# hugocornellier/face_detection_tflite

Measured on NVIDIA B200. Metric: images/sec BlazeFace detect (pre+infer+NMS), higher is better.
Workload: dtype f32

## Files before the change

face_detection_tflite_b200/csrc/engine.cu:

```cuda
#include "engine.h"

#include <algorithm>
#include <cstdio>
#include <cstdlib>

namespace fdt {

Engine::~Engine() {
  if (d_blob_) cudaFree(d_blob_);
  for (TailLayerD* p : d_tail_) if (p) cudaFree(p);
  for (TailBlk* p : d_blks_) if (p) cudaFree(p);
}

bool Engine::init(const uint8_t* tflite, size_t len, int fuse_level, std::string* err, bool use_tc) {
  if (!model_.parse(tflite, len, err)) return false;
  if (!plan_.build(model_, fuse_level, err, use_tc)) return false;
  size_t bytes = plan_.blob.size() * sizeof(float) + 64;
  if (cudaMalloc(&d_blob_, bytes) != cudaSuccess) { *err = "cudaMalloc(weights) failed"; return false; }
  cudaMemset(d_blob_, 0, bytes);
  if (cudaMemcpy(d_blob_, plan_.blob.data(), plan_.blob.size() * sizeof(float), cudaMemcpyHostToDevice) != cudaSuccess) {
    *err = "weight upload failed";
    return false;
  }
  d_tail_.assign(plan_.steps.size(), nullptr);
// ... 193 lines not shown
        p.no = st.no; p.KSo = st.KSo; p.out_stage_floats = st.out_stage_floats;
        p.out2 = nullptr; p.out2_istride = 0; p.Cs2 = 0; p.c1 = 0; p.c2 = 0;
        if (st.out2 >= 0) {
          TV o2 = view(ctx, st.out2);
          p.out2 = o2.p; p.out2_istride = o2.istride; p.Cs2 = o2.Cs; p.c1 = st.c1; p.c2 = st.c2;
          p.Cout = st.c1;
        }
        p.in_floats = st.in_stage_floats;
        if (!launch_block_ws(p, B, ctx.cap, s)) { failed_ = true; fprintf(stderr, "fdt: k_block_ws could not be launched for step '%s'\n", st.name.c_str()); }
        break;
      }
      case kStepTailWs: {
        TailP p;
        TV iv = view(ctx, st.in);
        p.in = iv.p; p.in_istride = iv.istride; p.H = iv.H; p.W = iv.W; p.CinS = iv.Cs;
        p.blob = blob; p.layers = d_tail_[&st - plan_.steps.data()]; p.nlayers = (int)st.tail.size();
        p.nbuf = st.tail_nbuf;
        for (int k = 0; k < kTailMaxBufs; ++k) { p.buf_off[k] = st.tail_buf_off[k]; p.buf_ks[k] = st.tail_buf_ks[k]; }
        p.act_floats = st.tail_act_floats; p.in_bytes = st.tail_in_bytes;
        p.generic = 0;
        for (const TailLayerD& L : st.tail)
          if (L.kind >= 2 || L.act == 2 || L.w_parts != 1 || L.wscale != 1.f || L.rbuf != L.src || (L.kind != 1 && L.o1 >= 0)) p.generic = 1;
        p.blks = nullptr; p.nblks = 0; p.bias_floats = 0; p.in_px = iv.H * iv.W;
        for (int k = 0; k < 2; ++k) { p.rsrc[k] = nullptr; p.rs_istride[k] = 0; p.rs_cs[k] = p.rs_w[k] = p.rs_c[k] = 0; }
        if (st.tail_wide) {
          p.generic = 2;
          p.blks = d_blks_[&st - plan_.steps.data()]; p.nblks = (int)st.tail_blks.size(); p.bias_floats = st.tail_bias_floats;
          for (size_t k = 0; k < st.tail_rsrc.size() && k < 2; ++k) {
            TV rv = view(ctx, st.tail_rsrc[k]);
            p.rsrc[k] = rv.p; p.rs_istride[k] = rv.istride; p.rs_cs[k] = rv.Cs; p.rs_w[k] = rv.W; p.rs_c[k] = rv.C;
          }
        }
        p.last_a_layer = st.tail_last_a; p.wbuf_bytes = st.tail_wbuf; p.wdepth = st.tail_wdepth; p.tbuf_bytes = st.tail_tbuf; p.smem_bytes = st.smem;
        for (int k = 0; k < 4; ++k) { p.outs[k] = nullptr; p.out_istride[k] = 0; p.out_pix[k] = 0; }
        for (size_t k = 0; k < st.tail_outs.size(); ++k) {
          TV ov = view(ctx, st.tail_outs[k]);
          p.outs[k] = ov.p; p.out_istride[k] = ov.istride; p.out_pix[k] = ov.Cs;
        }
        if (!launch_tail_ws(p, B, ctx.cap, s)) { failed_ = true; fprintf(stderr, "fdt: k_tail_ws could not be launched for step '%s'\n", st.name.c_str()); }
        break;
      }
      case kStepFcTc: {
        FcP p;
        TV iv = view(ctx, st.in);
        p.in = iv.p; p.in_istride = iv.istride;
        p.out = out.p; p.out_istride = out.istride;
        p.w = blob + st.w; p.bias = blob + st.bias;
        p.K = st.K; p.K16 = st.K8; p.N = st.Cout; p.w_parts = st.w_parts; p.tile_bytes = st.ts_rec_bytes; p.wscale = (float)st.out_scale;
        if (!launch_fc_tc(p, B, s)) { failed_ = true; fprintf(stderr, "fdt: k_fc_tc could not be launched for step '%s'\n", st.name.c_str()); }
        break;
      }
      case kStepBlockTs: {
        BlockTsP p;
        TV iv = view(ctx, st.in);
        p.in = iv.p; p.in_istride = iv.istride; p.H = iv.H; p.W = iv.W; p.CinS = iv.Cs;
        p.out = out.p; p.out_istride = out.istride; p.OH = out.H; p.OW = out.W; p.CoutS = out.Cs;
        p.rec = blob + st.ts_rec; p.bias = blob + st.ts_bias; p.rec_bytes = st.ts_rec_bytes;
        p.Cin = iv.C; p.K16 = st.ts_k16; p.Npad = st.ts_npad; p.KS = st.ts_ks;
        p.stride = st.dws; p.res = st.ts_res; p.relu = st.ts_relu;
        p.wide = (out.Cs % 8 == 0 && out.istride % 8 == 0 && ((size_t)out.p % 32 == 0)) ? 1 : 0;
        p.ns = st.ts_ns; p.stage_bytes = st.ts_stage_bytes; p.smem_bytes = st.smem;
        {
          const float* hdw = plan_.blob.data() + st.ts_rec + (size_t)st.ts_npad * st.ts_k16 / 2;
          for (int q = 0; q < 16; ++q)
            for (int k = 0; k < 10; ++k)
              for (int c = 0; c < 4; ++c) p.dw[(q * 10 + k) * 4 + c] = 4 * q + c < st.ts_k16 ? hdw[k * st.ts_k16 + 4 * q + c] : 0.f;
// ... 40 lines not shown
```

face_detection_tflite_b200/csrc/kernels.h:

```cpp
#pragma once
#include <cuda_runtime.h>
#include <algorithm>
#include <cstdint>

#include "../../include/fdt_api.h"
#include "tail_layer.h"

namespace fdt {

enum { kActNone = 0, kActRelu = 1, kActPrelu = 2 };

struct FastDiv {
  unsigned mul = 0, shr = 0, d = 1;
  FastDiv() {}
  explicit FastDiv(int div) {
    d = div < 1 ? 1u : (unsigned)div;
    unsigned l = 0;
    while ((1ull << l) < d) ++l;
    shr = l;
    mul = (unsigned)(((1ull << 32) * ((1ull << l) - d)) / d + 1);
  }
#ifdef __CUDACC__
  __device__ __forceinline__ int div(int n) const { return (int)((__umulhi(mul, (unsigned)n) + (unsigned)n) >> shr); }
  __device__ __forceinline__ void divmod(int n, int& q, int& r) const { q = div(n); r = n - q * (int)d; }
// ... 148 lines not shown
  float* out; long long out_istride; int OH, OW, CoutS;
  const float* rec;
  const float* bias;
  int rec_bytes;
  int Cin, K16, Npad, KS;
  int stride;
  int res;
  int relu, wide;
  int ns, stage_bytes;
  size_t smem_bytes;
  alignas(16) float dw[10 * 64];
};
size_t ts_smem_bytes(int rec_bytes, int Npad, int ns, int stage_bytes);
bool launch_block_ts(const BlockTsP& p, int B, int cap, cudaStream_t s);

struct TailP {
  const float* in; long long in_istride; int H, W, CinS;
  const float* blob;
  const TailLayerD* layers;
  int nlayers;
  int nbuf;
  int buf_off[kTailMaxBufs];
  int buf_ks[kTailMaxBufs];
  int act_floats;
  int in_bytes;
  int last_a_layer;
  int wbuf_bytes, wdepth;
  int tbuf_bytes;
  int generic;
  const TailBlk* blks; int nblks; int bias_floats; int in_px;
  const float* rsrc[2]; long long rs_istride[2]; int rs_cs[2], rs_w[2], rs_c[2];
  float* outs[4]; long long out_istride[4]; int out_pix[4];
  size_t smem_bytes;
};
size_t tail_smem_bytes(int act_floats, int wbuf_bytes, int wdepth, int tbuf_bytes);
size_t wide_smem_bytes(int act_floats, int wbuf_bytes, int wdepth, int tbuf_bytes, int bias_floats);
bool launch_tail_ws(const TailP& p, int B, int cap, cudaStream_t s);

struct FcP {
  const float* in; long long in_istride;
  float* out; long long out_istride;
  const float* w;
  const float* bias;
  int K, K16, N, w_parts, tile_bytes;
  float wscale;
};
bool launch_fc_tc(const FcP& p, int B, cudaStream_t s);

struct JpegIdctP {
  const int16_t* coef;
  const uint16_t* q;
  int bw, bh;
  uint8_t* plane; int pitch;
};
struct JpegColorP {
  const uint8_t* py; const uint8_t* pcb; const uint8_t* pcr;
  int pitch_y, pitch_c;
  int W, H, ncomp;
  int cdw, cdh, hs, vs;
  int orientation;
  uint8_t* out; int out_w;
};
void launch_jpeg_idct(const JpegIdctP& p, cudaStream_t s);
void launch_jpeg_color(const JpegColorP& p, cudaStream_t s);

struct DecodeP {
// ... 55 lines not shown
```

face_detection_tflite_b200/csrc/kernels_tail.cu:

```cuda
#include <cuda.h>
#include <cuda_fp16.h>

#include <algorithm>
#include <cstdio>
#include <map>
#include <mutex>
#include <tuple>

#include "kernels.h"

namespace fdt {
namespace {

#ifndef FDT_TAIL_WARPS
#define FDT_TAIL_WARPS 12
#endif
constexpr int kTC = FDT_TAIL_WARPS;
constexpr int kTG = kTC / 4;
constexpr int kTComputeThreads = kTC * 32;
constexpr int kTThreads = (kTC + 1) * 32;
__device__ __forceinline__ uint32_t col_d(int t) { return t ? 128u : 0u; }
__device__ __forceinline__ uint32_t col_a(int t) { return t ? 384u : 256u; }
constexpr uint32_t kLBO = 128;

// ... 25 lines not shown
}
__device__ __forceinline__ void fma4(float4& a, const float4& v, const float4& w) {
  asm("{\n\t.reg .b64 ra, rv, rw;\n\t"
      "mov.b64 ra, {%0, %1};\n\tmov.b64 rv, {%4, %5};\n\tmov.b64 rw, {%8, %9};\n\t"
      "fma.rn.f32x2 ra, rv, rw, ra;\n\tmov.b64 {%0, %1}, ra;\n\t"
      "mov.b64 ra, {%2, %3};\n\tmov.b64 rv, {%6, %7};\n\tmov.b64 rw, {%10, %11};\n\t"
      "fma.rn.f32x2 ra, rv, rw, ra;\n\tmov.b64 {%2, %3}, ra;\n\t}"
      : "+f"(a.x), "+f"(a.y), "+f"(a.z), "+f"(a.w)
      : "f"(v.x), "f"(v.y), "f"(v.z), "f"(v.w), "f"(w.x), "f"(w.y), "f"(w.z), "f"(w.w));
}
__device__ __forceinline__ float4 max4(const float4& a, const float4& b) {
  return make_float4(fmaxf(a.x, b.x), fmaxf(a.y, b.y), fmaxf(a.z, b.z), fmaxf(a.w, b.w));
}
__device__ __forceinline__ uint32_t pack_h2(float e0, float e1) {
  uint32_t d;
  asm("cvt.rn.satfinite.f16x2.f32 %0, %1, %2;" : "=r"(d) : "f"(e1), "f"(e0));
  return d;
}
__device__ __forceinline__ void split_store_tmem(uint32_t taddr_hi, const float4& a) {
  const uint32_t h0 = pack_h2(a.x, a.y), h1 = pack_h2(a.z, a.w);
  const __half2 hh0 = *reinterpret_cast<const __half2*>(&h0), hh1 = *reinterpret_cast<const __half2*>(&h1);
  const float2 f0 = __half22float2(hh0), f1 = __half22float2(hh1);
  const uint32_t l0 = pack_h2(a.x - f0.x, a.y - f0.y), l1 = pack_h2(a.z - f1.x, a.w - f1.y);
  asm volatile("tcgen05.st.sync.aligned.32x32b.x2.b32 [%0], {%1, %2};" ::"r"(taddr_hi), "r"(h0), "r"(h1) : "memory");
  asm volatile("tcgen05.st.sync.aligned.32x32b.x2.b32 [%0], {%1, %2};" ::"r"(taddr_hi + 64u), "r"(l0), "r"(l1) : "memory");
}
__device__ __forceinline__ void mma_ts_f16(uint32_t tmem_d, uint32_t tmem_a, uint32_t b_lo, uint32_t b_hi, uint32_t idesc, uint32_t acc) {
  asm volatile(
      "{\n\t.reg .pred p;\n\t.reg .b64 db;\n\tmov.b64 db, {%2, %3};\n\tsetp.ne.b32 p, %5, 0;\n\t"
      "tcgen05.mma.cta_group::1.kind::f16 [%0], [%1], db, %4, p;\n\t}\n" ::"r"(tmem_d), "r"(tmem_a), "r"(b_lo), "r"(b_hi), "r"(idesc), "r"(acc));
}

#ifdef FDT_TAIL_TRACE
#define TT(k) do { if (blockIdx.x == 0 && tid == 0 && it == 1) tt[l * 6 + (k)] = clock64(); } while (0)
#else
#define TT(k) do { } while (0)
#endif
template <bool GEN>
__global__ void __launch_bounds__(kTThreads, 1) k_tail_ws(const __grid_constant__ CUtensorMap tmap, const __grid_constant__ TailP p, int B) {
#ifdef FDT_TAIL_TRACE
  __shared__ long long tt[16 * 6];
#endif
  extern __shared__ __align__(128) unsigned char smem_raw[];
  __shared__ uint32_t tmem_base_s;
  const int tid = threadIdx.x, warp = tid >> 5, lane = tid & 31;
  TailLayerD* sL = reinterpret_cast<TailLayerD*>(smem_raw);
  float* sBias = reinterpret_cast<float*>(smem_raw + kTailMaxLayers * sizeof(TailLayerD));
  float* sAlpha = sBias + kTailMaxLayers * 128;
  uint64_t* bars = reinterpret_cast<uint64_t*>(sAlpha + kTailMaxLayers * 128);
  float* scratch = reinterpret_cast<float*>(bars + 16);
  float* act0 = reinterpret_cast<float*>((reinterpret_cast<uintptr_t>(scratch + 16) + 127) & ~(uintptr_t)127);
  float* zslot = act0 + p.act_floats;
  unsigned char* tring = reinterpret_cast<unsigned char*>((reinterpret_cast<uintptr_t>(zslot + 128) + 127) & ~(uintptr_t)127);
  unsigned char* wring = tring + 2 * (size_t)p.tbuf_bytes;
  const uint32_t bar0 = smem_u32(bars);
  const uint32_t in_full = bar0, a_free = bar0 + 8u, w_full = bar0 + 16u, a_full = bar0 + 32u, d_full = bar0 + 48u, t_full = bar0 + 56u;
  const int nl = p.nlayers;
  const int my_images = blockIdx.x < B ? (B - 1 - (int)blockIdx.x) / (int)gridDim.x + 1 : 0;

  for (int i = tid; i < nl * (int)(sizeof(TailLayerD) / 16); i += kTThreads)
    reinterpret_cast<uint4*>(sL)[i] = reinterpret_cast<const uint4*>(p.layers)[i];
  for (int i = (p.in_bytes >> 2) + tid; i < p.act_floats + 128; i += kTThreads) act0[i] = 0.f;
  if (warp == kTC) {
    if (lane == 0) {
      mbar_init(in_full, 1);
      mbar_init(a_free, kTC);
      for (int i = 0; i < 2; ++i) { mbar_init(w_full + 8u * i, 1); mbar_init(a_full + 8u * i, kTC); mbar_init(t_full + 8u * i, 1); }
      mbar_init(d_full, 1);
      asm volatile("fence.mbarrier_init.release.cluster;" ::: "memory");
      asm volatile("prefetch.tensormap [%0];" ::"l"(&tmap) : "memory");
    }
    __syncwarp();
    asm volatile("tcgen05.alloc.cta_group::1.sync.aligned.shared::cta.b32 [%0], %1;" ::"r"(smem_u32(&tmem_base_s)), "r"(512u));
    asm volatile("tcgen05.relinquish_alloc_permit.cta_group::1.sync.aligned;" ::);
  }
  __syncthreads();
  for (int l = 0; l < nl; ++l)
    for (int i = tid; i < sL[l].Npad; i += kTThreads) {
      sBias[l * 128 + i] = p.blob[(size_t)sL[l].bias_off + i];
      if (GEN && sL[l].act == 2) sAlpha[l * 128 + i] = p.blob[(size_t)sL[l].alpha_off + i];
    }
  asm volatile("tcgen05.fence::before_thread_sync;" ::: "memory");
  __syncthreads();
  asm volatile("tcgen05.fence::after_thread_sync;" ::: "memory");
  const uint32_t tmem_base = tmem_base_s;
  const uint32_t act_a = smem_u32(act0), zero_a = smem_u32(zslot), wring_a = smem_u32(wring), tring_a = smem_u32(tring);

  if (warp < kTC) {
    const int lq = warp & 3, g = warp >> 2;
    const int r = lq * 32 + lane;
    const uint32_t tm_lane = tmem_base + ((uint32_t)(lq * 32) << 16);
    uint32_t ph_d = 0u, ph_t0 = 0u, ph_t1 = 0u;
    int gl = 0, it = 0;
    for (int img = blockIdx.x; img < B; img += gridDim.x, ++it) {
      mbar_wait(in_full, (uint32_t)(it & 1));
      for (int l = 0; l < nl; ++l, ++gl) {
        const TailLayerD L = sL[l];
        TT(0);
        const uint32_t src_a = act_a + 4u * (uint32_t)p.buf_off[L.src], kss_b = 4u * (uint32_t)p.buf_ks[L.src];
        const uint32_t dst_a = L.dst >= 0 ? act_a + 4u * (uint32_t)p.buf_off[L.dst] : 0u, ksd_b = L.dst >= 0 ? 4u * (uint32_t)p.buf_ks[L.dst] : 0u;
        const int src_q = (int)(kss_b >> 4), dst_q = (int)(ksd_b >> 4);
        const int npix = L.OH * L.OW;
        const uint32_t tb_a = tring_a + (uint32_t)(gl & 1) * (uint32_t)p.tbuf_bytes;
        if (L.tap_bytes) {
          if (gl & 1) { mbar_wait(t_full + 8u, ph_t1); ph_t1 ^= 1u; } else { mbar_wait(t_full, ph_t0); ph_t0 ^= 1u; }
        }
        TT(1);
        if (GEN && L.kind == 3) {
          const int n = npix * L.Cin;
          float sacc = 0.f;
          for (int i = tid; i < n; i += kTComputeThreads) {
            const int px = i / L.Cin, c = i - px * L.Cin;
            float a, w;
            asm("ld.shared.f32 %0, [%1];" : "=f"(a) : "r"(src_a + (uint32_t)px * kss_b + 4u * (uint32_t)c) : "memory");
            asm("ld.shared.f32 %0, [%1];" : "=f"(w) : "r"(tb_a + 4u * (uint32_t)i) : "memory");
            sacc = fmaf(a, w, sacc);
          }
#pragma unroll
          for (int o = 16; o > 0; o >>= 1) sacc += __shfl_xor_sync(0xffffffffu, sacc, o);
          if (lane == 0) { scratch[warp] = sacc; mbar_arrive(a_full); mbar_arrive(a_full + 8u); }
          asm volatile("bar.sync 1, %0;" ::"n"(kTComputeThreads) : "memory");
          if (tid == 0) {
            float tot = sBias[l * 128];
            for (int w2 = 0; w2 < kTC; ++w2) tot += scratch[w2];
            p.outs[L.o1][(size_t)img * p.out_istride[L.o1]] = tot;
          }
          asm volatile("bar.sync 1, %0;" ::"n"(kTComputeThreads) : "memory");
          if (l == p.last_a_layer && lane == 0) mbar_arrive(a_free);
          continue;
        }
        const bool paired = npix > 128;
        const int ntiles = paired ? 2 : 1;
        const int rows = paired ? (npix >> 1) : npix;
        const int nq = L.K16 >> 2, nq_real = (L.Cin + 3) >> 2, nq_half = (L.K16 >> 5) << 2;
        const uint32_t dww_a = tb_a, dwb_a = dww_a + 9u * (uint32_t)L.K16 * 4u;
        const uint32_t k16_b = (uint32_t)L.K16 * 4u;
        const uint32_t acol0 = tm_lane + col_a(0), acol1 = tm_lane + col_a(1);
        int oy = r / L.OW;
        const int ox = r - oy * L.OW;
        if (paired) oy *= 2;
        const bool act = r < rows;
        const bool warp_on = lq * 32 < rows;
        const int pix0 = oy * L.OW + ox;
        bool half_done = false;
        if (!warp_on) {
        } else if (L.kind == 0) {
          uint32_t off[12];
          const int iy0 = oy * L.stride - L.pad, ix0 = ox * L.stride - L.pad;
#pragma unroll
          for (int k = 0; k < 12; ++k) {
            const int iy = iy0 + k / 3, ix = ix0 + k % 3;
            const bool ok = act && (unsigned)iy < (unsigned)L.IH && (unsigned)ix < (unsigned)L.IW;
            off[k] = ok ? src_a + (uint32_t)(iy * L.IW + ix) * kss_b : zero_a;
          }
          for (int q = g; q < nq; q += kTG) {
            if (!half_done && q >= nq_half) {
              half_done = true;
              asm volatile("tcgen05.wait::st.sync.aligned;" ::: "memory");
              asm volatile("tcgen05.fence::before_thread_sync;" ::: "memory");
              __syncwarp();
              if (lane == 0) mbar_arrive(a_full);
            }
            float4 a0 = make_float4(0.f, 0.f, 0.f, 0.f), a1 = a0;
            if (q < nq_real) {
              const uint32_t qo = 16u * (uint32_t)q;
              float4 w[9];
#pragma unroll
              for (int k = 0; k < 9; ++k) w[k] = lds4(dww_a + (uint32_t)k * k16_b + qo);
              const float4 bias = lds4(dwb_a + qo);
              float4 v[3];
#pragma unroll
              for (int c = 0; c < 3; ++c) v[c] = lds4(off[c] + qo);
              a0 = bias;
#pragma unroll
              for (int c = 0; c < 3; ++c) fma4(a0, v[c], w[c]);
// ... 26 lines not shown
              asm volatile("tcgen05.fence::before_thread_sync;" ::: "memory");
              __syncwarp();
              if (lane == 0) mbar_arrive(a_full);
            }
            const bool in = q < src_q;
            split_store_tmem(acol0 + 2u * (uint32_t)q, in ? lds4(px0 + 16u * (uint32_t)q) : make_float4(0.f, 0.f, 0.f, 0.f));
            if (paired) split_store_tmem(acol1 + 2u * (uint32_t)q, in ? lds4(px1 + 16u * (uint32_t)q) : make_float4(0.f, 0.f, 0.f, 0.f));
          }
        }
        if (warp_on) asm volatile("tcgen05.wait::st.sync.aligned;" ::: "memory");
        TT(2);
        asm volatile("tcgen05.fence::before_thread_sync;" ::: "memory");
        __syncwarp();
        if (lane == 0) { if (!half_done) mbar_arrive(a_full); mbar_arrive(a_full + 8u); }
        if (warp_on) {
          const uint32_t bias_a = smem_u32(sBias + l * 128), alpha_a = smem_u32(sAlpha + l * 128);
          const uint32_t rsrc_a = GEN ? act_a + 4u * (uint32_t)p.buf_off[L.rbuf] : src_a, ksr_b = GEN ? 4u * (uint32_t)p.buf_ks[L.rbuf] : kss_b;
          const int res_q = (int)(ksr_b >> 4);
          mbar_wait(d_full, ph_d);
          TT(3);
          asm volatile("tcgen05.fence::after_thread_sync;" ::: "memory");
          const uint32_t row_b = (uint32_t)L.IW * ksr_b;
#pragma unroll 1
          for (int t = 0; t < ntiles; ++t) {
            const int pix = pix0 + t * L.OW;
            const uint32_t dcol = tm_lane + col_d(t);
            uint32_t res_a = zero_a;
            if (act && L.res == 1) res_a = rsrc_a + (uint32_t)pix * ksr_b;
            if (act && L.res == 2) res_a = rsrc_a + (uint32_t)((2 * oy) * L.IW + 2 * ox) * ksr_b;
            const uint32_t out_a = dst_a + (uint32_t)(act ? pix : 0) * ksd_b;
            float* o1 = nullptr; float* o2 = nullptr;
            int o1_q = 0;
            if (GEN ? L.o1 >= 0 : L.kind == 1) {
              o1 = p.outs[L.o1] + (size_t)img * p.out_istride[L.o1] + (size_t)(act ? pix : 0) * p.out_pix[L.o1];
              o1_q = p.out_pix[L.o1] >> 2;
              if (L.o2 >= 0) o2 = p.outs[L.o2] + (size_t)img * p.out_istride[L.o2] + (size_t)(act ? pix : 0) * p.out_pix[L.o2];
            }
            for (int c16 = g; c16 < (L.Npad >> 4); c16 += kTG) {
              uint32_t u[16];
              asm volatile(
                  "tcgen05.ld.sync.aligned.32x32b.x16.b32 {%0, %1, %2, %3, %4, %5, %6, %7, %8, %9, %10, %11, %12, %13, %14, %15}, [%16];"
                  : "=r"(u[0]), "=r"(u[1]), "=r"(u[2]), "=r"(u[3]), "=r"(u[4]), "=r"(u[5]), "=r"(u[6]), "=r"(u[7]),
                    "=r"(u[8]), "=r"(u[9]), "=r"(u[10]), "=r"(u[11]), "=r"(u[12]), "=r"(u[13]), "=r"(u[14]), "=r"(u[15])
                  : "r"(dcol + 16u * (uint32_t)c16));
              float4 bv[4], rv[4];
#pragma unroll
              for (int j = 0; j < 4; ++j) {
                const int cq = 4 * c16 + j;
                const uint32_t qo = 16u * (uint32_t)cq;
                bv[j] = lds4(bias_a + qo);
                rv[j] = make_float4(0.f, 0.f, 0.f, 0.f);
                if (L.res == 1) {
                  if (cq < res_q) rv[j] = lds4(res_a + qo);
                } else if (L.res == 2) {
                  if (cq < res_q) rv[j] = max4(max4(lds4(res_a + qo), lds4(res_a + ksr_b + qo)), max4(lds4(res_a + row_b + qo), lds4(res_a + row_b + ksr_b + qo)));
                }
              }
              asm volatile("tcgen05.wait::ld.sync.aligned;" ::: "memory");
#pragma unroll
              for (int j = 0; j < 4; ++j) {
                const int cq = 4 * c16 + j;
                float4 v;
                if (GEN) v = make_float4(fmaf(__uint_as_float(u[4 * j]), L.wscale, bv[j].x), fmaf(__uint_as_float(u[4 * j + 1]), L.wscale, bv[j].y),
                                         fmaf(__uint_as_float(u[4 * j + 2]), L.wscale, bv[j].z), fmaf(__uint_as_float(u[4 * j + 3]), L.wscale, bv[j].w));
                else v = make_float4(__uint_as_float(u[4 * j]) + bv[j].x, __uint_as_float(u[4 * j + 1]) + bv[j].y,
                                     __uint_as_float(u[4 * j + 2]) + bv[j].z, __uint_as_float(u[4 * j + 3]) + bv[j].w);
                if (L.kind != 1) {
                  v.x += rv[j].x; v.y += rv[j].y; v.z += rv[j].z; v.w += rv[j].w;
                  if (L.act == 1) {
                    v = max4(v, make_float4(0.f, 0.f, 0.f, 0.f));
                  } else if (GEN && L.act == 2) {
                    const float4 al = lds4(alpha_a + 16u * (uint32_t)cq);
                    v = make_float4(fmaf(al.x, fminf(v.x, 0.f), fmaxf(v.x, 0.f)), fmaf(al.y, fminf(v.y, 0.f), fmaxf(v.y, 0.f)),
                                    fmaf(al.z, fminf(v.z, 0.f), fmaxf(v.z, 0.f)), fmaf(al.w, fminf(v.w, 0.f), fmaxf(v.w, 0.f)));
                  }
                  if (act && cq < dst_q) sts4(out_a + 16u * (uint32_t)cq, v);
                  if (GEN && act && cq < o1_q) *reinterpret_cast<float4*>(o1 + 4 * cq) = v;
                } else if (act) {
                  const int c = 4 * cq;
                  if (c + 4 <= L.c1) {
                    *reinterpret_cast<float4*>(o1 + c) = v;
                  } else {
                    const float vv[4] = {v.x, v.y, v.z, v.w};
#pragma unroll
                    for (int e = 0; e < 4; ++e)
                      if (c + e >= L.c1 && c + e - L.c1 < L.c2) o2[c + e - L.c1] = vv[e];
                  }
                }
              }
            }
          }
        }
        ph_d ^= 1u;
        TT(4);
        asm volatile("tcgen05.fence::before_thread_sync;" ::: "memory");
        asm volatile("bar.sync 1, %0;" ::"n"(kTComputeThreads) : "memory");
        TT(5);
        asm volatile("tcgen05.fence::after_thread_sync;" ::: "memory");
        if (l == p.last_a_layer && lane == 0) mbar_arrive(a_free);
      }
#ifdef FDT_TAIL_TRACE
      if (blockIdx.x == 0 && tid == 0 && it == 1)
        for (int l2 = 0; l2 < nl; ++l2)
          printf("tail layer %2d: taps-wait %5lld  depthwise %6lld  mma-wait %5lld  epilogue %5lld  barrier %5lld  | total %6lld\n", l2, tt[l2 * 6 + 1] - tt[l2 * 6],
                 tt[l2 * 6 + 2] - tt[l2 * 6 + 1], tt[l2 * 6 + 3] - tt[l2 * 6 + 2], tt[l2 * 6 + 4] - tt[l2 * 6 + 3], tt[l2 * 6 + 5] - tt[l2 * 6 + 4],
                 tt[l2 * 6 + 5] - tt[l2 * 6]);
#endif
    }
  } else if (lane == 0) {
    const int total = my_images * nl;
    const int D = p.wdepth;
    auto load_weights = [&](int glayer) {
      const TailLayerD& L = sL[glayer % nl];
      if (!L.rec_bytes) return;
      const uint32_t slot = (uint32_t)(glayer % D), bar = w_full + 8u * slot;
      mbar_expect_tx(bar, (uint32_t)L.rec_bytes);
      asm volatile("cp.async.bulk.shared::cluster.global.mbarrier::complete_tx::bytes [%0], [%1], %2, [%3];"
                   ::"r"(wring_a + slot * (uint32_t)p.wbuf_bytes), "l"(p.blob + (size_t)L.rec_off), "r"((uint32_t)L.rec_bytes), "r"(bar) : "memory");
    };
    auto load_taps = [&](int glayer) {
      const TailLayerD& L = sL[glayer % nl];
      if (!L.tap_bytes) return;
      const uint32_t slot = (uint32_t)(glayer & 1), bar = t_full + 8u * slot;
      mbar_expect_tx(bar, (uint32_t)L.tap_bytes);
      asm volatile("cp.async.bulk.shared::cluster.global.mbarrier::complete_tx::bytes [%0], [%1], %2, [%3];"
                   ::"r"(tring_a + slot * (uint32_t)p.tbuf_bytes), "l"(p.blob + (size_t)L.tap_off), "r"((uint32_t)L.tap_bytes), "r"(bar) : "memory");
    };
    auto load_image = [&](int img) {
      mbar_expect_tx(in_full, (uint32_t)p.in_bytes);
      asm volatile("cp.async.bulk.tensor.4d.shared::cluster.global.mbarrier::complete_tx::bytes [%0], [%1, {%2, %3, %4, %5}], [%6];"
                   ::"r"(act_a), "l"(&tmap), "r"(0), "r"(0), "r"(0), "r"(img), "r"(in_full) : "memory");
    };
    if (my_images > 0) {
      load_image(blockIdx.x);
      for (int i = 0; i < D && i < total; ++i) load_weights(i);
      for (int i = 0; i < 2 && i < total; ++i) load_taps(i);
    }
    uint32_t ph_a = 0u, ph_d = 0u, ph_w0 = 0u, ph_w1 = 0u;
    int gl = 0, it = 0;
    for (int img = blockIdx.x; img < B; img += gridDim.x, ++it) {
      for (int l = 0; l < nl; ++l, ++gl) {
        const TailLayerD& L = sL[l];
        if (!GEN || L.kind != 3) {
          const int ntiles = L.OH * L.OW > 128 ? 2 : 1;
          const uint32_t idesc = (1u << 4) | ((uint32_t)(L.Npad >> 3) << 17) | ((128u >> 4) << 24);
          const uint32_t sbo = (uint32_t)(L.K16 >> 3) * 128u;
          const uint32_t b_hi = ((sbo >> 4) & 0x3FFFu) | (1u << 14);
          const int slot = gl % D;
          const uint32_t wb_a = wring_a + (uint32_t)slot * (uint32_t)p.wbuf_bytes;
          const uint32_t b_lo0 = ((wb_a & 0x3FFFFu) >> 4) | ((kLBO >> 4) << 16);
          const uint32_t b_lo1 = (((wb_a + (uint32_t)(L.Npad * L.K16) * 2u) & 0x3FFFFu) >> 4) | ((kLBO >> 4) << 16);
          const int ksteps = L.K16 >> 4, khalf = L.K16 >> 5;
          if (slot) { mbar_wait_idle(w_full + 8u, ph_w1); ph_w1 ^= 1u; } else { mbar_wait_idle(w_full, ph_w0); ph_w0 ^= 1u; }
          for (int half = 0; half < 2; ++half) {
            mbar_wait_idle(a_full + 8u * (uint32_t)half, ph_a);
            asm volatile("tcgen05.fence::after_thread_sync;" ::: "memory");
            const int k0 = half ? khalf : 0, k1 = half ? ksteps : khalf;
            for (int t = 0; t < ntiles; ++t) {
              const uint32_t dcol = tmem_base + col_d(t), acol = tmem_base + col_a(t);
#pragma unroll 1
              for (int ks = k0; ks < k1; ++ks) {
                mma_ts_f16(dcol, acol + 8u * (uint32_t)ks, b_lo0 + 16u * (uint32_t)ks, b_hi, idesc, ks ? 1u : 0u);
                mma_ts_f16(dcol, acol + 64u + 8u * (uint32_t)ks, b_lo0 + 16u * (uint32_t)ks, b_hi, idesc, 1u);
                if (GEN && L.w_parts == 2) mma_ts_f16(dcol, acol + 8u * (uint32_t)ks, b_lo1 + 16u * (uint32_t)ks, b_hi, idesc, 1u);
              }
            }
          }
          ph_a ^= 1u;
          asm volatile("tcgen05.commit.cta_group::1.mbarrier::arrive::one.shared::cluster.b64 [%0];" ::"r"(d_full) : "memory");
          mbar_wait_idle(d_full, ph_d);
          ph_d ^= 1u;
        } else {
          mbar_wait_idle(a_full, ph_a);
          mbar_wait_idle(a_full + 8u, ph_a);
          ph_a ^= 1u;
        }
        if (gl + D < total) load_weights(gl + D);
        if (gl + 2 < total) load_taps(gl + 2);
        if (l == p.last_a_layer && img + (int)gridDim.x < B) {
          mbar_wait_idle(a_free, (uint32_t)(it & 1));
          load_image(img + (int)gridDim.x);
        }
      }
    }
  }
  __syncwarp();
  asm volatile("tcgen05.fence::before_thread_sync;" ::: "memory");
  __syncthreads();
  if (warp == kTC) {
    asm volatile("tcgen05.fence::after_thread_sync;" ::: "memory");
    asm volatile("tcgen05.dealloc.cta_group::1.sync.aligned.b32 %0, %1;" ::"r"(tmem_base), "r"(512u));
  }
}


constexpr int kWThreads = (kTC + 2) * 32;
constexpr int kWideZero = 512;
__global__ void __launch_bounds__(kWThreads, 1) k_chain_wide(const __grid_constant__ TailP p, int B) {
  extern __shared__ __align__(128) unsigned char smem_raw[];
  __shared__ uint32_t tmem_base_s;
  const int tid = threadIdx.x, warp = tid >> 5, lane = tid & 31;
  TailLayerD* sL = reinterpret_cast<TailLayerD*>(smem_raw);
  TailBlk* sBlk = reinterpret_cast<TailBlk*>(smem_raw + kTailMaxLayers * sizeof(TailLayerD));
  float* sBias = reinterpret_cast<float*>(sBlk + kTailMaxBlks);
  float* sAlpha = sBias + p.bias_floats;
  uint64_t* bars = reinterpret_cast<uint64_t*>(sAlpha + p.bias_floats);
  float* scratch = reinterpret_cast<float*>(bars + 32);
  float* act0 = reinterpret_cast<float*>((reinterpret_cast<uintptr_t>(scratch + 16) + 127) & ~(uintptr_t)127);
  float* zslot = act0 + p.act_floats;
  unsigned char* tring = reinterpret_cast<unsigned char*>((reinterpret_cast<uintptr_t>(zslot + kWideZero) + 127) & ~(uintptr_t)127);
  unsigned char* wring = tring + 2 * (size_t)p.tbuf_bytes;
  const uint32_t bar0 = smem_u32(bars);
  const uint32_t in_full = bar0, a_free = bar0 + 8u, a_full = bar0 + 16u, d_full = bar0 + 32u, t_full = bar0 + 40u, a_done = bar0 + 56u,
                 w_full = bar0 + 64u, w_free = bar0 + 96u;
  const int nl = p.nlayers;
  const int my_images = blockIdx.x < B ? (B - 1 - (int)blockIdx.x) / (int)gridDim.x + 1 : 0;
// ... 479 lines not shown
```

face_detection_tflite_b200/csrc/plan.cpp:

```cpp
#include "plan.h"

#include <algorithm>
#include <cmath>
#include <cstdio>
#include <cstdlib>
#include <cstring>
#include <cstdint>

namespace fdt {
namespace {

constexpr size_t kSmemLimit = 200 * 1024;
constexpr int kActNone = 0, kActRelu = 1, kActPrelu = 2;

inline int ru(int v, int m) { return (v + m - 1) / m * m; }
inline int smem_stride(int KP) { return KP + (((KP / 4) % 2 == 0) ? 4 : 0); }

void same_pad(int in, int k, int s, int* before) {
  int out = (in + s - 1) / s;
  int total = (out - 1) * s + k - in;
  if (total < 0) total = 0;
  *before = total / 2;
}

// ... 881 lines not shown
      wbuf = std::max(wbuf, (size_t)L.rec_bytes);
      tbuf = std::max(tbuf, (size_t)L.tap_bytes);
      if (L.rec_bytes % 16 || L.tap_bytes % 16) return false;
      if (L.src == 0 || L.dst == 0 || (L.res && L.rbuf == 0)) last0 = (int)li;
    }
    t->tail_last_a = last0;
    t->tail_tbuf = (int)((tbuf + 127) / 128 * 128);
    if (t->tail_wide) {
      int need = 2;
      for (const TailLayerD& L : t->tail) need = std::max(need, L.ng >> 8);
      for (const TailBlk& b : t->tail_blks) wbuf = std::max(wbuf, (size_t)b.bytes);
      t->tail_wbuf = (int)((wbuf + 127) / 128 * 128);
      if (t->tail_blks.size() > (size_t)kTailMaxBlks) return false;
      auto wbytes = [&](int depth) {
        return (size_t)kTailMaxLayers * sizeof(TailLayerD) + (size_t)kTailMaxBlks * sizeof(TailBlk) + 2 * (size_t)t->tail_bias_floats * 4 + 32 * 8 + 16 * 4 + 128 +
               ((size_t)off + 512) * 4 + 128 + 2 * (size_t)t->tail_tbuf + (size_t)depth * t->tail_wbuf;
      };
      int depth = 4;
      while (depth > need && wbytes(depth) > (size_t)225 * 1024) --depth;
      t->tail_wdepth = depth;
      t->smem = wbytes(depth);
      return t->smem <= (size_t)225 * 1024;
    }
    t->tail_wbuf = (int)((wbuf + 127) / 128 * 128);
    auto bytes = [&](int depth) {
      return (size_t)kTailMaxLayers * sizeof(TailLayerD) + 2 * (size_t)kTailMaxLayers * 512 + 16 * 8 + 16 * 4 + 128 +
             ((size_t)off + 128) * 4 + 128 + 2 * (size_t)t->tail_tbuf + (size_t)depth * t->tail_wbuf;
    };
    t->tail_wdepth = bytes(2) <= (size_t)225 * 1024 ? 2 : 1;
    t->smem = bytes(t->tail_wdepth);
    return t->smem <= (size_t)225 * 1024;
  }

  void redo_liveness() {
    for (PTensor& x : P.tensors) { x.materialized = false; x.def_step = -1; x.last_use = -1; }
    for (size_t i = 0; i < P.steps.size(); ++i) {
      const PStep& s = P.steps[i];
      P.tensors[s.out].materialized = true;
      if (s.out2 >= 0) P.tensors[s.out2].materialized = true;
      for (int e : s.extra_out) { P.tensors[e].materialized = true; use((int)i, e); }
      for (int e : s.tail_rsrc) use((int)i, e);
      if (!s.in_u8) use((int)i, s.in);
      use((int)i, s.in2);
      use((int)i, s.out);
      use((int)i, s.out2);
    }
  }

  void fuse_tail() {
    const int S = (int)P.steps.size();
    auto block_ok = [&](const PStep& s) {
      if ((s.kind != kStepBlockWs && s.kind != kStepBlockTs) || s.w_parts != 1 || s.in < 0) return false;
      const PTensor& in = P.tensors[s.in];
      const PTensor& out = P.tensors[s.out];
      if (in.H * in.W > 256 || in.root >= 0 || in.C > 128 || s.Cout > 128) return false;
      if (s.has_dw) {
        if (s.c2 > 0 || out.root >= 0 || (s.act != kActRelu && s.act != kActNone)) return false;
        if (s.in2 >= 0 && (s.res_mode != 1 || s.in2 != s.in)) return false;
        if (s.dws != 1 && s.dws != 2) return false;
        if (s.dws == 2 && (in.H % 2 || in.W % 2 || s.dpt != 0 || s.dpl != 0)) return false;
        if (s.dws == 1 && (s.dpt != 1 || s.dpl != 1)) return false;
        return true;
      }
      if (s.in2 >= 0 || s.act != kActNone || out.root < 0) return false;
      if (s.c2 > 0 ? (s.c1 % 4 != 0 || s.out2 < 0 || P.tensors[s.out2].root < 0) : (s.Cout % 4 != 0)) return false;
      return true;
// ... 60 lines not shown
      } else {
        L.dst = -1;
        L.c1 = s.c2 > 0 ? s.c1 : s.Cout; L.c2 = s.c2;
        L.o1 = (int)t.tail_outs.size(); t.tail_outs.push_back(s.out);
        if (s.c2 > 0) { L.o2 = (int)t.tail_outs.size(); t.tail_outs.push_back(s.out2); }
        if (t.tail_outs.size() > 4) return;
      }
      if (!(L.OH * L.OW <= 128 || (L.OH * L.OW <= 256 && L.OH % 2 == 0 && (!s.has_dw || s.dws == 1)))) return;
      const size_t SBO8 = (size_t)(s.K8 / 4) * 128;
      const int K16 = L.K16;
      std::vector<float> wplain((size_t)s.Cout * in.C);
      for (int n = 0; n < s.Cout; ++n)
        for (int k = 0; k < in.C; ++k)
          wplain[(size_t)n * in.C + k] = P.blob[(size_t)s.w + ((size_t)(n >> 3) * SBO8 + (size_t)(k >> 2) * 128 + (size_t)(n & 7) * 16 + (size_t)(k & 3) * 4) / 4];
      if (!f16_exact(wplain)) return;
      std::vector<float> rec = pack_w_f16(wplain, s.Cout, in.C, L.Npad, K16, 1, &L.wscale);
      L.rec_bytes = (int)(rec.size() * 4);
      L.rec_off = (int)push(rec, rec.size());
      if (s.has_dw) {
        std::vector<float> dw((size_t)10 * K16, 0.f);
        for (int k = 0; k < 9; ++k)
          for (int c = 0; c < in.C; ++c) dw[(size_t)k * K16 + c] = P.blob[(size_t)s.dww + (size_t)k * s.K8 + c];
        for (int c = 0; c < in.C; ++c) dw[(size_t)9 * K16 + c] = P.blob[(size_t)s.dwb + c];
        L.tap_bytes = (int)(dw.size() * 4);
        L.tap_off = (int)push(dw, dw.size());
      }
      std::vector<float> bias((size_t)L.Npad, 0.f);
      for (int n = 0; n < s.Cout; ++n) bias[n] = P.blob[(size_t)s.bias + n];
      L.bias_off = (int)push(bias, bias.size());
      t.macs += s.macs;
      t.tail.push_back(L);
    }
    if (t.tail_outs.empty() || !finish_tail(&t, {PA, PB}, {maxA, maxB})) return;
    t.in = X;
    t.out = t.tail_outs[0];
    for (size_t k = 1; k < t.tail_outs.size(); ++k) t.extra_out.push_back(t.tail_outs[k]);
    t.name = "tail:" + P.steps[order.front()].name + ".." + P.steps[order.back()].name;
    P.steps.resize(f);
    P.steps.push_back(t);
    redo_liveness();
  }

  struct ChainOut { int emit_at; PStep step; };
  std::vector<ChainOut> chains;
  void fuse_chain() {
    static const int want = [] { const char* e = std::getenv("FDT_CHAIN"); return e ? std::atoi(e) : 1; }();
    if (!want) return;
    bool narrow_done = false;
    for (size_t s0 = 0; s0 < m.ops.size(); ++s0)
      if (m.ops[s0].code == kOpConv2D && !done[s0]) try_chain((int)s0, &narrow_done);
  }

  struct ChainLayer { int conv; PwMatch M; int kind; int out_tf; };

  std::vector<float> pack_w_block(const std::vector<float>& w, int N, int K, int n0, int ncols, int k0, int kw, int parts, float scale) {
    const size_t SBO16 = (size_t)(kw / 8) * 128;
    std::vector<uint16_t> img((size_t)parts * ncols * kw, 0);
    for (int n = 0; n < ncols && n0 + n < N; ++n)
      for (int k = 0; k < kw && k0 + k < K; ++k) {
        const float v = w[(size_t)(n0 + n) * K + k0 + k] * scale;
        const size_t o = ((size_t)(n >> 3) * SBO16 + (size_t)(k >> 3) * 128 + (size_t)(n & 7) * 16 + (size_t)(k & 7) * 2) / 2;
        const uint16_t hb = f32_to_f16(v);
        img[o] = hb;
        if (parts == 2) img[(size_t)ncols * kw + o] = f32_to_f16(v - f16_to_f32(hb));
      }
    std::vector<float> rec((img.size() + 1) / 2, 0.f);
// ... 490 lines not shown
    }
    P.arena_per_image = top;
    return true;
  }
};

}

bool Plan::build(const TfModel& m, int fuse, std::string* err, bool use_tc) {
  *this = Plan();
  fuse_level = fuse;
  Builder b(m, *this, fuse);
  b.use_tc = use_tc;
  bool ok = b.run();
  if (!ok && err) *err = b.err;
  return ok;
}

std::string Plan::describe() const {
  static const char* kn[] = {"normalize", "naive_conv", "gemm_conv", "dwpw", "add", "act", "padc", "maxpool", "resize", "stem", "block_ws", "stem_ws", "tail_ws", "fc_tc", "block_ts"};
  std::string s;
  char buf[512];
  double macs = 0;
  for (size_t i = 0; i < steps.size(); ++i) {
    const PStep& st = steps[i];
    const PTensor& o = tensors[st.out];
    macs += st.macs;
    snprintf(buf, sizeof buf,
             "%3zu %-10s in=%d res=%d%s/m%d out=%d[%dx%dx%d Cs%d %s] act=%d dw=%d/s%d K=%d NC=%dx%d TM=%d NPG=%d tile=%dx%dx%d RS=%d nd=%d ns=%d na=%d no=%d smem=%zu  %s\n",
             i, kn[st.kind], st.in >= 0 ? tensors[st.in].tf : -1, st.in2 >= 0 ? tensors[st.in2].tf : -1,
             st.res_pool ? "(pool)" : "", st.res_mode, o.tf, o.H, o.W, o.C, o.Cs, o.root >= 0 ? "view" : "arena", st.act,
             (int)st.has_dw, st.dws, st.K, st.NC, st.nchunks, st.TM, st.NPG, st.TH, st.TW, st.G, st.RS, st.nd, st.ns, st.na, st.no, st.smem, st.name.c_str());
    s += buf;
    if (st.kind == kStepBlockWs && (st.nr > 0 || st.deint)) {
      snprintf(buf, sizeof buf, "      k_block_ws: residual ring %d x %d B (record %d floats)%s\n", st.nr, st.res_stage_floats * 4, st.KSr,
               st.deint ? ", stride 2 on even / odd column planes" : "");
      s += buf;
    }
    if (st.tail_wide) {
      snprintf(buf, sizeof buf, "      k_chain_wide: %zu W blocks (ring %d x %d B), act %d floats, %zu HBM residual tensor(s)\n", st.tail_blks.size(), st.tail_wdepth, st.tail_wbuf,
               st.tail_act_floats, st.tail_rsrc.size());
      s += buf;
    }
    for (size_t l = 0; l < st.tail.size(); ++l) {
      const TailLayerD& L = st.tail[l];
      static const char* lk[] = {"block", "heads", "pw", "dot"};
      snprintf(buf, sizeof buf, "      tail %2zu %s buf %d->%d %dx%d->%dx%d s%d C %d->%d K16=%d Npad=%d res=%d(buf %d) act=%d wparts=%d out=%d rec=%dB taps=%dB\n", l, lk[L.kind & 3],
               L.src, L.dst, L.IH, L.IW, L.OH, L.OW, L.stride, L.Cin, L.Cout, L.K16, L.Npad, L.res, L.rbuf, L.act, L.w_parts, L.o1, L.rec_bytes, L.tap_bytes);
      s += buf;
      if (st.tail_wide && L.kind != 3) {
        s.pop_back();
        snprintf(buf, sizeof buf, " wide: groups=%d blocks/group=%d Kchunks=%d blk0=%d\n", L.ng & 0xff, L.ng >> 8, L.nk, L.blk0);
        s += buf;
      }
    }
  }
  snprintf(buf, sizeof buf, "steps=%zu  MACs/image=%.3fM  arena/image=%.1f KB  weights=%.1f KB\n", steps.size(),
           macs / 1e6, arena_per_image * 4.0 / 1024, blob.size() * 4.0 / 1024);
  s += buf;
  return s;
}

}
```

face_detection_tflite_b200/csrc/plan.h:

```cpp
#pragma once
#include <map>
#include <string>
#include <vector>

#include "tail_layer.h"
#include "tflite_model.h"

namespace fdt {

struct PTensor {
  int tf = -1;
  int H = 1, W = 1, C = 1, Cs = 1;
  long long istride = 0;
  int root = -1;
  long long view_off = 0;
  long long arena_off = -1;
  int def_step = -1, last_use = -1;
  bool materialized = false;
  bool is_input = false;
};

enum StepKind { kStepNormalize, kStepNaiveConv, kStepGemmConv, kStepDwPw, kStepAdd, kStepAct, kStepPadC,
                kStepMaxPool, kStepResize, kStepStem, kStepBlockWs, kStepStemWs, kStepTailWs, kStepFcTc, kStepBlockTs };

struct PStep {
  StepKind kind = kStepAct;
  std::string name;
  int in = -1, in2 = -1, out = -1;
  int kh = 1, kw = 1, sh = 1, sw = 1, pt = 0, pl = 0, act = 0, depthwise = 0;
  bool in_u8 = false;
  bool has_dw = false;
  int dws = 1, dpt = 0, dpl = 0, res_pool = 0, res_mode = 0;
  long long w = -1, bias = -1, alpha = -1, dww = -1, dwb = -1;
  int K = 0, KP = 0, KS = 0, Cout = 0, CoutP = 0, NC = 0, nchunks = 0, NPG = 0, TM = 0;
  int TH = 0, TW = 0, G = 1, IH = 0, IW = 0, tilesX = 1, tilesY = 1;
  size_t smem = 0;
  int K8 = 0, Npad = 0, a_rows = 0, RS = 1, tmem_cols = 0, w_parts = 1, nbuf = 1;
  double out_scale = 1.0;
  int ns = 0, na = 0, nd = 8, nt = 2, in_stage_floats = 0;
  int no = 0, KSo = 0, out_stage_floats = 0;
  int nr = 0, KSr = 0, res_stage_floats = 0;
  int deint = 0, plane_floats = 0, PW = 0;
  int out2 = -1, c1 = 0, c2 = 0;
  int fh = 1, fw = 1, align = 0, half = 0;
  std::vector<int> extra_out;
  long long ts_rec = -1, ts_bias = -1;
  int ts_rec_bytes = 0, ts_k16 = 0, ts_npad = 0, ts_ks = 0, ts_ns = 0, ts_stage_bytes = 0, ts_res = 0, ts_relu = 0;
  std::vector<TailLayerD> tail;
  std::vector<int> tail_outs;
  int tail_nbuf = 0, tail_buf_off[kTailMaxBufs] = {0}, tail_buf_ks[kTailMaxBufs] = {0}, tail_buf_px[kTailMaxBufs] = {0};
  std::vector<TailBlk> tail_blks;
  std::vector<int> tail_rsrc;
  int tail_wide = 0, tail_bias_floats = 0;
  int tail_act_floats = 0, tail_in_bytes = 0, tail_last_a = 0, tail_wbuf = 0, tail_wdepth = 2, tail_tbuf = 0;
  double macs = 0;
};

struct Plan {
  std::vector<PTensor> tensors;
  std::vector<PStep> steps;
  std::vector<float> blob;
  std::map<int, int> tf2pt;
  int input = -1, in_h = 0, in_w = 0;
  std::vector<int> outputs;
  std::vector<long long> out_elems;
  long long arena_per_image = 0;
  int fuse_level = 1;

  bool build(const TfModel& m, int fuse_level, std::string* err, bool use_tc = true);
  std::string describe() const;
};

}
```

Measured before the change: 774,500.

## Pair two images through the small tail layers to fill 128-row MMA tiles

After the single stride-2 layer of the tail chain, activations have at most 64 pixels, so each MMA tile is half empty. The tail kernel now processes two images per iteration: it runs the front layers separately for image A and image B, then runs the post-stride layers once with rows 0-63 for A and 64-127 for B. The plan allocates a doubled buffer for this and keeps pairing only when shared memory and ring depth still fit. The cost is more complex scheduling of weight and tap loads and of the mbarrier phases, plus larger shared memory, and the path is limited to the non-generic kernel variant.

```diff
diff --git a/face_detection_tflite_b200/csrc/engine.cu b/face_detection_tflite_b200/csrc/engine.cu
--- a/face_detection_tflite_b200/csrc/engine.cu
+++ b/face_detection_tflite_b200/csrc/engine.cu
@@ -249,6 +249,7 @@
           }
         }
         p.last_a_layer = st.tail_last_a; p.wbuf_bytes = st.tail_wbuf; p.wdepth = st.tail_wdepth; p.tbuf_bytes = st.tail_tbuf; p.smem_bytes = st.smem;
+        p.pair_from = p.generic ? -1 : st.tail_pair_from; p.pair_stride = st.tail_pair_stride;
         for (int k = 0; k < 4; ++k) { p.outs[k] = nullptr; p.out_istride[k] = 0; p.out_pix[k] = 0; }
         for (size_t k = 0; k < st.tail_outs.size(); ++k) {
           TV ov = view(ctx, st.tail_outs[k]);
diff --git a/face_detection_tflite_b200/csrc/kernels.h b/face_detection_tflite_b200/csrc/kernels.h
--- a/face_detection_tflite_b200/csrc/kernels.h
+++ b/face_detection_tflite_b200/csrc/kernels.h
@@ -204,6 +204,7 @@
   const float* rsrc[2]; long long rs_istride[2]; int rs_cs[2], rs_w[2], rs_c[2];
   float* outs[4]; long long out_istride[4]; int out_pix[4];
   size_t smem_bytes;
+  int pair_from, pair_stride;
 };
 size_t tail_smem_bytes(int act_floats, int wbuf_bytes, int wdepth, int tbuf_bytes);
 size_t wide_smem_bytes(int act_floats, int wbuf_bytes, int wdepth, int tbuf_bytes, int bias_floats);
diff --git a/face_detection_tflite_b200/csrc/kernels_tail.cu b/face_detection_tflite_b200/csrc/kernels_tail.cu
--- a/face_detection_tflite_b200/csrc/kernels_tail.cu
+++ b/face_detection_tflite_b200/csrc/kernels_tail.cu
@@ -81,14 +81,14 @@
 }
 
 #ifdef FDT_TAIL_TRACE
-#define TT(k) do { if (blockIdx.x == 0 && tid == 0 && it == 1) tt[l * 6 + (k)] = clock64(); } while (0)
+#define TT(k) do { if (blockIdx.x == 0 && tid == 0 && it == (GEN ? 1 : 0)) tt[s * 6 + (k)] = clock64(); } while (0)
 #else
 #define TT(k) do { } while (0)
 #endif
 template <bool GEN>
 __global__ void __launch_bounds__(kTThreads, 1) k_tail_ws(const __grid_constant__ CUtensorMap tmap, const __grid_constant__ TailP p, int B) {
 #ifdef FDT_TAIL_TRACE
-  __shared__ long long tt[16 * 6];
+  __shared__ long long tt[2 * kTailMaxLayers * 6];
 #endif
   extern __shared__ __align__(128) unsigned char smem_raw[];
   __shared__ uint32_t tmem_base_s;
@@ -106,6 +106,7 @@
   const uint32_t in_full = bar0, a_free = bar0 + 8u, w_full = bar0 + 16u, a_full = bar0 + 32u, d_full = bar0 + 48u, t_full = bar0 + 56u;
   const int nl = p.nlayers;
   const int my_images = blockIdx.x < B ? (B - 1 - (int)blockIdx.x) / (int)gridDim.x + 1 : 0;
+  const int pf = GEN ? -1 : p.pair_from;
 
   for (int i = tid; i < nl * (int)(sizeof(TailLayerD) / 16); i += kTThreads)
     reinterpret_cast<uint4*>(sL)[i] = reinterpret_cast<const uint4*>(p.layers)[i];
@@ -140,14 +141,23 @@
     const int r = lq * 32 + lane;
     const uint32_t tm_lane = tmem_base + ((uint32_t)(lq * 32) << 16);
     uint32_t ph_d = 0u, ph_t0 = 0u, ph_t1 = 0u;
-    int gl = 0, it = 0;
-    for (int img = blockIdx.x; img < B; img += gridDim.x, ++it) {
-      mbar_wait(in_full, (uint32_t)(it & 1));
-      for (int l = 0; l < nl; ++l, ++gl) {
+    int gl = 0, it = 0, nin = 0;
+    for (int img = blockIdx.x; img < B; ++it) {
+      const bool has_b = !GEN && pf >= 0 && img + (int)gridDim.x < B;
+      const int len = has_b ? nl + pf : nl;
+      for (int s = 0; s < len; ++s, ++gl) {
+        const int part = has_b ? (s < pf ? 0 : s < 2 * pf ? 1 : 2) : 0;
+        const int l = part ? s - pf : s;
         const TailLayerD L = sL[l];
         TT(0);
-        const uint32_t src_a = act_a + 4u * (uint32_t)p.buf_off[L.src], kss_b = 4u * (uint32_t)p.buf_ks[L.src];
-        const uint32_t dst_a = L.dst >= 0 ? act_a + 4u * (uint32_t)p.buf_off[L.dst] : 0u, ksd_b = L.dst >= 0 ? 4u * (uint32_t)p.buf_ks[L.dst] : 0u;
+        if (s == 0 || (part == 1 && s == pf)) { mbar_wait(in_full, (uint32_t)(nin & 1)); ++nin; }
+        const bool pp = part == 2;
+        const int slot = pp ? r >> 6 : part;
+        const int rr = pp ? (r & 63) : r;
+        const int oimg = slot ? img + (int)gridDim.x : img;
+        const uint32_t sofs = 4u * (uint32_t)(slot * p.pair_stride);
+        const uint32_t src_a = act_a + 4u * (uint32_t)p.buf_off[L.src] + (L.src == 1 ? sofs : 0u), kss_b = 4u * (uint32_t)p.buf_ks[L.src];
+        const uint32_t dst_a = L.dst >= 0 ? act_a + 4u * (uint32_t)p.buf_off[L.dst] + (L.dst == 1 ? sofs : 0u) : 0u, ksd_b = L.dst >= 0 ? 4u * (uint32_t)p.buf_ks[L.dst] : 0u;
         const int src_q = (int)(kss_b >> 4), dst_q = (int)(ksd_b >> 4);
         const int npix = L.OH * L.OW;
         const uint32_t tb_a = tring_a + (uint32_t)(gl & 1) * (uint32_t)p.tbuf_bytes;
@@ -185,11 +195,11 @@
         const uint32_t dww_a = tb_a, dwb_a = dww_a + 9u * (uint32_t)L.K16 * 4u;
         const uint32_t k16_b = (uint32_t)L.K16 * 4u;
         const uint32_t acol0 = tm_lane + col_a(0), acol1 = tm_lane + col_a(1);
-        int oy = r / L.OW;
-        const int ox = r - oy * L.OW;
+        int oy = rr / L.OW;
+        const int ox = rr - oy * L.OW;
         if (paired) oy *= 2;
-        const bool act = r < rows;
-        const bool warp_on = lq * 32 < rows;
+        const bool act = rr < rows;
+        const bool warp_on = (pp ? (lq & 1) : lq) * 32 < rows;
         const int pix0 = oy * L.OW + ox;
         bool half_done = false;
         if (!warp_on) {
@@ -282,9 +292,9 @@
             float* o1 = nullptr; float* o2 = nullptr;
             int o1_q = 0;
             if (GEN ? L.o1 >= 0 : L.kind == 1) {
-              o1 = p.outs[L.o1] + (size_t)img * p.out_istride[L.o1] + (size_t)(act ? pix : 0) * p.out_pix[L.o1];
+              o1 = p.outs[L.o1] + (size_t)oimg * p.out_istride[L.o1] + (size_t)(act ? pix : 0) * p.out_pix[L.o1];
               o1_q = p.out_pix[L.o1] >> 2;
-              if (L.o2 >= 0) o2 = p.outs[L.o2] + (size_t)img * p.out_istride[L.o2] + (size_t)(act ? pix : 0) * p.out_pix[L.o2];
+              if (L.o2 >= 0) o2 = p.outs[L.o2] + (size_t)oimg * p.out_istride[L.o2] + (size_t)(act ? pix : 0) * p.out_pix[L.o2];
             }
             for (int c16 = g; c16 < (L.Npad >> 4); c16 += kTG) {
               uint32_t u[16];
@@ -350,18 +360,28 @@
         if (l == p.last_a_layer && lane == 0) mbar_arrive(a_free);
       }
 #ifdef FDT_TAIL_TRACE
-      if (blockIdx.x == 0 && tid == 0 && it == 1)
-        for (int l2 = 0; l2 < nl; ++l2)
-          printf("tail layer %2d: taps-wait %5lld  depthwise %6lld  mma-wait %5lld  epilogue %5lld  barrier %5lld  | total %6lld\n", l2, tt[l2 * 6 + 1] - tt[l2 * 6],
-                 tt[l2 * 6 + 2] - tt[l2 * 6 + 1], tt[l2 * 6 + 3] - tt[l2 * 6 + 2], tt[l2 * 6 + 4] - tt[l2 * 6 + 3], tt[l2 * 6 + 5] - tt[l2 * 6 + 4],
-                 tt[l2 * 6 + 5] - tt[l2 * 6]);
+      if (blockIdx.x == 0 && tid == 0 && it == (GEN ? 1 : 0))
+        for (int s2 = 0; s2 < len; ++s2) {
+          const int part = has_b ? (s2 < pf ? 0 : s2 < 2 * pf ? 1 : 2) : 0;
+          printf("tail pass %2d (layer %2d, %s): in+taps-wait %5lld  depthwise %6lld  mma-wait %5lld  epilogue %5lld  barrier %5lld  | total %6lld\n", s2,
+                 part ? s2 - pf : s2, part == 0 ? (has_b ? "a  " : "one") : part == 1 ? "b  " : "a+b", tt[s2 * 6 + 1] - tt[s2 * 6],
+                 tt[s2 * 6 + 2] - tt[s2 * 6 + 1], tt[s2 * 6 + 3] - tt[s2 * 6 + 2], tt[s2 * 6 + 4] - tt[s2 * 6 + 3], tt[s2 * 6 + 5] - tt[s2 * 6 + 4],
+                 tt[s2 * 6 + 5] - tt[s2 * 6]);
+        }
 #endif
+      img += has_b ? 2 * (int)gridDim.x : (int)gridDim.x;
     }
   } else if (lane == 0) {
-    const int total = my_images * nl;
+    const int npairs = pf >= 0 ? my_images / 2 : 0;
+    const int pair_total = npairs * (nl + pf);
+    const int total = pair_total + (my_images - 2 * npairs) * nl;
+    auto layer_of = [&](int g) {
+      if (!GEN && g < pair_total) { const int s = g % (nl + pf); return s < pf ? s : s - pf; }
+      return (g - pair_total) % nl;
+    };
     const int D = p.wdepth;
     auto load_weights = [&](int glayer) {
-      const TailLayerD& L = sL[glayer % nl];
+      const TailLayerD& L = sL[layer_of(glayer)];
       if (!L.rec_bytes) return;
       const uint32_t slot = (uint32_t)(glayer % D), bar = w_full + 8u * slot;
       mbar_expect_tx(bar, (uint32_t)L.rec_bytes);
@@ -369,7 +389,7 @@
                    ::"r"(wring_a + slot * (uint32_t)p.wbuf_bytes), "l"(p.blob + (size_t)L.rec_off), "r"((uint32_t)L.rec_bytes), "r"(bar) : "memory");
     };
     auto load_taps = [&](int glayer) {
-      const TailLayerD& L = sL[glayer % nl];
+      const TailLayerD& L = sL[layer_of(glayer)];
       if (!L.tap_bytes) return;
       const uint32_t slot = (uint32_t)(glayer & 1), bar = t_full + 8u * slot;
       mbar_expect_tx(bar, (uint32_t)L.tap_bytes);
@@ -388,8 +408,12 @@
     }
     uint32_t ph_a = 0u, ph_d = 0u, ph_w0 = 0u, ph_w1 = 0u;
     int gl = 0, it = 0;
-    for (int img = blockIdx.x; img < B; img += gridDim.x, ++it) {
-      for (int l = 0; l < nl; ++l, ++gl) {
+    for (int img = blockIdx.x; img < B;) {
+      const bool has_b = !GEN && pf >= 0 && img + (int)gridDim.x < B;
+      const int len = has_b ? nl + pf : nl;
+      for (int s = 0; s < len; ++s, ++gl) {
+        const int part = has_b ? (s < pf ? 0 : s < 2 * pf ? 1 : 2) : 0;
+        const int l = part ? s - pf : s;
         const TailLayerD& L = sL[l];
         if (!GEN || L.kind != 3) {
           const int ntiles = L.OH * L.OW > 128 ? 2 : 1;
@@ -427,11 +451,16 @@
         }
         if (gl + D < total) load_weights(gl + D);
         if (gl + 2 < total) load_taps(gl + 2);
-        if (l == p.last_a_layer && img + (int)gridDim.x < B) {
-          mbar_wait_idle(a_free, (uint32_t)(it & 1));
-          load_image(img + (int)gridDim.x);
+        if (l == p.last_a_layer && part < 2) {
+          const int cur = part ? img + (int)gridDim.x : img;
+          if (cur + (int)gridDim.x < B) {
+            mbar_wait_idle(a_free, (uint32_t)(it & 1));
+            load_image(cur + (int)gridDim.x);
+          }
+          ++it;
         }
       }
+      img += has_b ? 2 * (int)gridDim.x : (int)gridDim.x;
     }
   }
   __syncwarp();
diff --git a/face_detection_tflite_b200/csrc/plan.cpp b/face_detection_tflite_b200/csrc/plan.cpp
--- a/face_detection_tflite_b200/csrc/plan.cpp
+++ b/face_detection_tflite_b200/csrc/plan.cpp
@@ -937,6 +937,23 @@
     return t->smem <= (size_t)225 * 1024;
   }
 
+  void pair_tail(PStep* t, int PA, int PB, int maxA, int maxB) {
+    const int n = (int)t->tail.size();
+    int s2 = -1, n_s2 = 0;
+    for (int li = 0; li < n; ++li)
+      if (t->tail[li].kind == 0 && t->tail[li].stride == 2) { s2 = li; ++n_s2; }
+    if (n_s2 != 1 || s2 + 1 >= n || t->tail[s2].dst != 1 || t->tail_last_a != s2 || PB > 64) return;
+    for (int li = s2 + 1; li < n; ++li) {
+      const TailLayerD& L = t->tail[li];
+      if (L.src != 1 || (L.dst != 1 && L.dst != -1) || (L.res && L.rbuf != 1) || L.IH * L.IW > 64 || L.OH * L.OW > 64) return;
+    }
+    PStep u = *t;
+    if (!finish_tail(&u, {PA, 2 * PB}, {maxA, maxB}) || u.tail_wdepth != t->tail_wdepth) return;
+    u.tail_pair_from = s2 + 1;
+    u.tail_pair_stride = PB * u.tail_buf_ks[1];
+    *t = u;
+  }
+
   void redo_liveness() {
     for (PTensor& x : P.tensors) { x.materialized = false; x.def_step = -1; x.last_use = -1; }
     for (size_t i = 0; i < P.steps.size(); ++i) {
@@ -1063,6 +1080,7 @@
       t.tail.push_back(L);
     }
     if (t.tail_outs.empty() || !finish_tail(&t, {PA, PB}, {maxA, maxB})) return;
+    pair_tail(&t, PA, PB, maxA, maxB);
     t.in = X;
     t.out = t.tail_outs[0];
     for (size_t k = 1; k < t.tail_outs.size(); ++k) t.extra_out.push_back(t.tail_outs[k]);
@@ -1619,6 +1637,11 @@
              st.res_pool ? "(pool)" : "", st.res_mode, o.tf, o.H, o.W, o.C, o.Cs, o.root >= 0 ? "view" : "arena", st.act,
              (int)st.has_dw, st.dws, st.K, st.NC, st.nchunks, st.TM, st.NPG, st.TH, st.TW, st.G, st.RS, st.nd, st.ns, st.na, st.no, st.smem, st.name.c_str());
     s += buf;
+    if (st.kind == kStepTailWs) {
+      s.pop_back();
+      snprintf(buf, sizeof buf, " pair=%d\n", st.tail_pair_from);
+      s += buf;
+    }
     if (st.kind == kStepBlockWs && (st.nr > 0 || st.deint)) {
       snprintf(buf, sizeof buf, "      k_block_ws: residual ring %d x %d B (record %d floats)%s\n", st.nr, st.res_stage_floats * 4, st.KSr,
                st.deint ? ", stride 2 on even / odd column planes" : "");
diff --git a/face_detection_tflite_b200/csrc/plan.h b/face_detection_tflite_b200/csrc/plan.h
--- a/face_detection_tflite_b200/csrc/plan.h
+++ b/face_detection_tflite_b200/csrc/plan.h
@@ -53,6 +53,7 @@
   std::vector<int> tail_rsrc;
   int tail_wide = 0, tail_bias_floats = 0;
   int tail_act_floats = 0, tail_in_bytes = 0, tail_last_a = 0, tail_wbuf = 0, tail_wdepth = 2, tail_tbuf = 0;
+  int tail_pair_from = -1, tail_pair_stride = 0;
   double macs = 0;
 };
 
```

After: 789,300, median of 6. 1.02x the previous value.
